# fmazilu/ASR-using-robust-NN

Hardware: AMD Instinct MI355X
Metric: utterances/sec (train, 1 s@16 kHz) (higher is better)
Workload: dtype f32 accumulate, fp16 two-plane split products in the training GEMMs (22-bit operands); 1 GPU; raw 16 kHz waveform -> on-GPU MFCC -> Lipschitz-constrained MLP train step (Adam+NonNeg, simple_norm_constraint rho=0.1), 1xMI355X; global_batch=1024, per_gpu_batch=1024, clip=1 s @ 16 kHz fp32, resident_pool_clips_per_gpu=65536, parallelism=dp1, hip_graph=False

## Files before the change

asr-using-robust-nn_amd/csrc/common.h:

```cpp
#pragma once
#include <hip/hip_runtime.h>
#include <cstdarg>
#include <cstdio>
#include <cstring>
#include <cmath>
#include <algorithm>
#include <vector>
#include "../../include/lipasr.h"

namespace lipasr {

void set_error(const char* fmt, ...);

#define LP_CHECK_ARG(cond, ...)                    \
  do {                                             \
    if (!(cond)) {                                 \
      lipasr::set_error(__VA_ARGS__);              \
      return LIPASR_EINVAL;                        \
    }                                              \
  } while (0)

#define LP_HIP(expr)                                                                   \
  do {                                                                                 \
    hipError_t _e = (expr);                                                            \
    if (_e != hipSuccess) {                                                            \
      lipasr::set_error("%s failed: %s (%s:%d)", #expr, hipGetErrorString(_e), __FILE__, __LINE__); \
      return LIPASR_EHIP;                                                              \
    }                                                                                  \
  } while (0)

#define LP_LAUNCH_CHECK() LP_HIP(hipGetLastError())

bool ensure_dyn_lds(const void* fn, size_t bytes);
int device_cus();
// ... 85 lines not shown
```

asr-using-robust-nn_amd/csrc/core.hip:

```cpp
#include "common.h"
#include <map>
#include <mutex>

namespace lipasr {

static thread_local char g_err[512] = "";

void set_error(const char* fmt, ...) {
  va_list ap;
  va_start(ap, fmt);
  vsnprintf(g_err, sizeof(g_err), fmt, ap);
  va_end(ap);
}

int device_cus() {
  static int cached[16] = {};
  int dev = 0; (void)hipGetDevice(&dev);
  int& c = cached[dev & 15];
  if (!c) { hipDeviceProp_t prop; c = hipGetDeviceProperties(&prop, dev) == hipSuccess ? prop.multiProcessorCount : 256; }
  return c;
}

bool ensure_dyn_lds(const void* fn, size_t bytes) {
  if (bytes <= 48 * 1024) return true;
  struct Limit { size_t granted = 0, refused = SIZE_MAX; };
  static std::mutex mu;
  static std::map<std::pair<const void*, int>, Limit> limits;
  int dev = 0; (void)hipGetDevice(&dev);
  std::lock_guard<std::mutex> lock(mu);
  Limit& l = limits[{fn, dev}];
  if (bytes <= l.granted) return true;
  if (bytes >= l.refused) return false;
  if (hipFuncSetAttribute(fn, hipFuncAttributeMaxDynamicSharedMemorySize, (int)bytes) == hipSuccess) { l.granted = bytes; return true; }
  set_error("hipFuncSetAttribute: %zu bytes of dynamic LDS refused: %s", bytes, hipGetErrorString(hipGetLastError()));
  l.refused = bytes;
  return false;
}

void mfcc_plan_free(MfccPlan* p);
void mlp_plan_free(lipasr_mlp* m);

}

using namespace lipasr;

extern "C" {

int lipasr_version(void) { return 560; }

const char* lipasr_last_error(void) { return g_err; }

int lipasr_create(int device, lipasr_handle_t* out) {
  LP_CHECK_ARG(out != nullptr, "lipasr_create: out is null");
  int n = 0;
  LP_HIP(hipGetDeviceCount(&n));
  LP_CHECK_ARG(device >= 0 && device < n, "lipasr_create: device %d out of range (have %d)", device, n);
  hipDeviceProp_t prop;
  LP_HIP(hipGetDeviceProperties(&prop, device));
  if (strncmp(prop.gcnArchName, "gfx950", 6) != 0) {
    set_error("lipasr_create: device %d is %s; this library is built for gfx950 only", device, prop.gcnArchName);
    return LIPASR_EUNSUPPORTED;
  }
  DeviceGuard g(device);
  if (!g.ok) { set_error("lipasr_create: hipSetDevice(%d) failed", device); return LIPASR_EHIP; }
  lipasr_ctx* c = new lipasr_ctx();
  c->device = device;
  c->scratch_floats = kScratchFloats;
  if (hipMalloc(&c->scratch, c->scratch_floats * sizeof(float)) != hipSuccess) {
    delete c;
    set_error("lipasr_create: scratch allocation failed");
    return LIPASR_ENOMEM;
// ... 55 lines not shown
  LP_HIP(hipEventRecord(h->timers[2 * id], S(stream)));
  return LIPASR_OK;
}

int lipasr_timer_stop(lipasr_handle_t h, int id, lipasr_stream_t stream) {
  LP_CHECK_ARG(h && id >= 0 && (size_t)(2 * id + 1) < h->timers.size(), "lipasr_timer_stop: bad timer id %d", id);
  LP_HIP(hipEventRecord(h->timers[2 * id + 1], S(stream)));
  return LIPASR_OK;
}

int lipasr_timer_elapsed_ms(lipasr_handle_t h, int id, float* ms_host) {
  LP_CHECK_ARG(h && ms_host && id >= 0 && (size_t)(2 * id + 1) < h->timers.size(),
               "lipasr_timer_elapsed_ms: bad argument");
  LP_HIP(hipEventSynchronize(h->timers[2 * id + 1]));
  LP_HIP(hipEventElapsedTime(ms_host, h->timers[2 * id], h->timers[2 * id + 1]));
  return LIPASR_OK;
}

namespace lipasr {
constexpr long long kFlagHardFactor = 4;
__global__ void flag_signal_kernel(int* flag, int value) {
  if (threadIdx.x == 0) __hip_atomic_store(flag, value, __ATOMIC_RELEASE, __HIP_MEMORY_SCOPE_AGENT);
}
__global__ void flag_wait_kernel(const int* flag, int value, int* err, long long soft_ticks) {
  if (threadIdx.x == 0) {
    const long long t0 = wall_clock64();
    bool reported = false;
    while (__hip_atomic_load(flag, __ATOMIC_ACQUIRE, __HIP_MEMORY_SCOPE_AGENT) < value) {
      __builtin_amdgcn_s_sleep(16);
      const long long dt = wall_clock64() - t0;
      if (!reported && dt > soft_ticks) {
        if (__hip_atomic_load(err, __ATOMIC_RELAXED, __HIP_MEMORY_SCOPE_SYSTEM) >= 2) break;
        __hip_atomic_store(err, 1, __ATOMIC_RELAXED, __HIP_MEMORY_SCOPE_SYSTEM);
        reported = true;
      }
      if (dt > kFlagHardFactor * soft_ticks) { __hip_atomic_store(err, 2, __ATOMIC_RELAXED, __HIP_MEMORY_SCOPE_SYSTEM); break; }
    }
  }
}
}

int lipasr_flag_signal(lipasr_handle_t h, int* flag, int value, lipasr_stream_t stream) {
  LP_CHECK_ARG(h && flag, "lipasr_flag_signal: null argument");
  hipLaunchKernelGGL(lipasr::flag_signal_kernel, dim3(1), dim3(64), 0, S(stream), flag, value);
  LP_LAUNCH_CHECK();
  return LIPASR_OK;
}

int lipasr_flag_wait(lipasr_handle_t h, const int* flag, int value, int timeout_ms, int* err, lipasr_stream_t stream) {
  LP_CHECK_ARG(h && flag && err, "lipasr_flag_wait: null argument");
  LP_CHECK_ARG(timeout_ms >= 1 && timeout_ms <= 150000, "lipasr_flag_wait: timeout %d ms outside [1, 150000]", timeout_ms);
  hipLaunchKernelGGL(lipasr::flag_wait_kernel, dim3(1), dim3(64), 0, S(stream), flag, value, err, (long long)timeout_ms * 100000LL);
  LP_LAUNCH_CHECK();
  return LIPASR_OK;
}

int lipasr_graph_begin(lipasr_handle_t h, lipasr_stream_t stream) {
  LP_CHECK_ARG(h != nullptr, "lipasr_graph_begin: null handle");
  LP_HIP(hipStreamBeginCapture(S(stream), hipStreamCaptureModeThreadLocal));
  return LIPASR_OK;
}

int lipasr_graph_end(lipasr_handle_t h, lipasr_stream_t stream, int* graph_id) {
  LP_CHECK_ARG(h && graph_id, "lipasr_graph_end: null argument");
  hipGraph_t graph = nullptr;
  LP_HIP(hipStreamEndCapture(S(stream), &graph));
  hipGraphExec_t exec = nullptr;
  hipError_t e = hipGraphInstantiate(&exec, graph, nullptr, nullptr, 0);
  (void)hipGraphDestroy(graph);
  if (e != hipSuccess) {
    set_error("hipGraphInstantiate failed: %s", hipGetErrorString(e));
// ... 49 lines not shown
```

asr-using-robust-nn_amd/csrc/gemm.hip:

```cpp
#include "gemm.h"
#include <algorithm>
#include <cstdint>

namespace lipasr {

static GemmKnobs g_knobs;
const GemmKnobs& gemm_knobs() { return g_knobs; }
constexpr int kEpiCount = EPI_DH_BNX + 1;
static long g_gemm_launches[GK_KINDS][2][2][2][3][kEpiCount] = {};
static long g_group_launches[3][3] = {};
static long g_group_ring_problems[4] = {};
static long g_group_ring_launches[4] = {};

static int arith_index(int bf16) { return bf16 == 2 ? 2 : bf16 == 1 ? 1 : 0; }
static const GemmTable& gemm_table() { static const GemmTable t; return t; }

static GemmPick gemm_instance(int kind, bool exchange, int amode, int bmode, int ar) {
  const GemmTable& t = gemm_table();
  const GemmShape& s = t.shape[kind];
  return GemmPick{kind, s.tile_m, s.tile_n, s.threads, s.lds_bytes, t.fn[kind][exchange ? 1 : 0][amode][bmode][ar]};
}

static bool aligned16(const void* p) { return (reinterpret_cast<uintptr_t>(p) & 15) == 0; }
static bool ring_legal(int amode, int bmode, const GemmArgs& g) {
// ... 167 lines not shown
using namespace lipasr;

extern "C" {

long lipasr_debug_gemm_launches(int kind, int exchange, int amode, int bmode, int arith, int epi) {
  if (kind < 0 || kind >= GK_KINDS || (exchange | amode | bmode) & ~1 || arith < 0 || arith > 2 || epi < -1 || epi >= kEpiCount) return -1;
  if (!gemm_table().fn[kind][exchange][amode][bmode][arith]) return -1;
  const long* c = g_gemm_launches[kind][exchange][amode][bmode][arith];
  if (epi >= 0) return c[epi];
  long n = 0;
  for (int e = 0; e < kEpiCount; ++e) n += c[e];
  return n;
}

long lipasr_debug_group_launches(int family, int arith, int variant) {
  if (family < 0 || family > 2 || arith < 0 || arith > 2) return -1;
  if (family < 2) return variant == -1 ? g_group_launches[family][arith] : -1;
  if (arith != 2 || variant < -1 || variant > 3) return -1;
  return variant == -1 ? g_group_launches[2][2] : g_group_ring_problems[variant];
}

long lipasr_debug_launch_count(int kind) {
  if (kind == 0) return lipasr_debug_gemm_launches(GK_RING2, 1, 0, 0, 2, -1) + lipasr_debug_gemm_launches(GK_RING2, 1, 0, 1, 2, -1);
  return kind == 1 ? g_group_ring_launches[2] : -1;
}

int lipasr_debug_gemm_mode(int mode) {
  GemmKnobs k;
  k.gemm_mode = mode & 3;
  k.split_dw0 = (mode >> 2) & 1;
  k.group_lds = !((mode >> 3) & 1);
  k.xcd_map = (mode >> 4) & 1;
  k.no_ring = (mode >> 5) & 1;
  k.ring_tile = ((mode >> 6) & 1) ? 1 : ((mode >> 7) & 1) ? 3 : 2;
  k.ring2 = !((mode >> 8) & 1);
  k.ring_x1 = !((mode >> 9) & 1);
  g_knobs = k;
  return LIPASR_OK;
}

static int gemm_entry(const char* fn, lipasr_handle_t h, int arith, int transA, int transB, int M, int N, int K, const float* A, int lda,
                      const float* B, int ldb, float* C, int ldc, float scale_a, float scale_b, lipasr_stream_t stream) {
  LP_CHECK_ARG(h && A && B && C, "%s: null argument", fn);
  LP_CHECK_ARG(arith >= 0 && arith <= 2, "%s: arithmetic mode %d (0 = exact fp32, 1 = bf16 operands, 2 = fp16 two-plane split)", fn, arith);
  LP_CHECK_ARG(M > 0 && N > 0 && K > 0, "%s: empty problem %dx%dx%d", fn, M, N, K);
  LP_CHECK_ARG(lda >= (transA ? M : K) && ldb >= (transB ? K : N) && ldc >= N, "%s: leading dimension too small", fn);
// ... 30 lines not shown
```

asr-using-robust-nn_amd/csrc/stft_bdft.hip:

```cpp
#include "stft.h"

namespace lipasr {

using namespace tables;

typedef _Float16 bd_h8 __attribute__((ext_vector_type(8)));
typedef _Float16 bd_h2 __attribute__((ext_vector_type(2)));
typedef float bd_f2 __attribute__((ext_vector_type(2)));
typedef float bd_f32x16 __attribute__((ext_vector_type(16)));

constexpr int kBdPlane = 1028;
constexpr int kBdSlot = 2 * kBdPlane;
constexpr int kBdSlots = 7;
constexpr int kBdTwF4 = 16 * 64;
constexpr int kBdLdsFloats = kBdSlots * kBdSlot + 4 * kBdTwF4;
constexpr int kBdDummy = 2048;
constexpr double kBdSig = 2048.0, kBdTap = 64.0, kBdMid = 1.0 / 1024.0;
constexpr float kBdOut = 8192.0f;

struct BdftArgs {
  StftArgs st;
  const uint4* cfrag;
  const uint4* efrag;
  const float4* tw;
  const float* wlo;
  const float* whi;
  const unsigned long long* smask;
  const int4* mpos;
  int seg_frames;
  int L;
  const float4* dct_frag;
  const double* aff_mean;
  const double* aff_scale;
  float* out;
};

__device__ __forceinline__ void bd_split8(const float (&x)[8], bd_h8& hi, bd_h8& lo) {
  unsigned h[4], l[4];
#pragma unroll
  for (int i = 0; i < 4; ++i) h[i] = __builtin_bit_cast(unsigned, __builtin_convertvector((bd_f2){x[2 * i], x[2 * i + 1]}, bd_h2));
  asm("v_fma_mixlo_f16 %0, %4, 1.0, -%12 op_sel_hi:[0,0,1]\n\t"
// ... 190 lines not shown
    float pl_, ph_;
    if (j == 0) {
      pl_ = 0.0f; ph_ = 0.0f;
    } else {
      asm("v_cndmask_b32 %0, %1, 0, %2" : "=v"(pl_) : "v"(cl_), "s"(sm[j]));
      asm("v_cndmask_b32 %0, %1, 0, %2" : "=v"(ph_) : "v"(ch_), "s"(sm[j]));
    }
    cl_ = fmaf(wl[j], pw[j], pl_);
    ch_ = fmaf(wh[j], pw[j], ph_);
    sl[j] = cl_; sh[j] = ch_;
  }
}

__device__ __forceinline__ void bd_load_weights(const BdftArgs& a, int lane, float (&wl)[16], float (&wh)[16]) {
#pragma unroll
  for (int q = 0; q < 4; ++q) {
    const float4 l4 = reinterpret_cast<const float4*>(a.wlo)[4 * lane + q], h4 = reinterpret_cast<const float4*>(a.whi)[4 * lane + q];
    wl[4 * q] = l4.x; wl[4 * q + 1] = l4.y; wl[4 * q + 2] = l4.z; wl[4 * q + 3] = l4.w;
    wh[4 * q] = h4.x; wh[4 * q + 1] = h4.y; wh[4 * q + 2] = h4.z; wh[4 * q + 3] = h4.w;
  }
}

__device__ __forceinline__ float bd_frame_finish(const BdftArgs& a, float* __restrict__ stg, const float (&sl)[16], const float (&sh)[16],
                                                 const unsigned (&mp)[6], int lane, int u, int f) {
  const int x = (lane >> 2) & 3;
#pragma unroll
  for (int q = 0; q < 4; ++q) {
    *reinterpret_cast<float4*>(stg + 16 * lane + 4 * (q ^ x)) = make_float4(sl[4 * q], sl[4 * q + 1], sl[4 * q + 2], sl[4 * q + 3]);
    *reinterpret_cast<float4*>(stg + 1024 + 16 * lane + 4 * (q ^ x)) = make_float4(sh[4 * q], sh[4 * q + 1], sh[4 * q + 2], sh[4 * q + 3]);
  }
  if (lane == 0) stg[kBdDummy] = 0.0f;
  const float m0 = ((stg[mp[0] & 0xffff] + stg[mp[0] >> 16]) + stg[mp[1] & 0xffff]) + ((stg[mp[1] >> 16] + stg[mp[2] & 0xffff]) + stg[mp[2] >> 16]);
  const float m1 = ((stg[mp[3] & 0xffff] + stg[mp[3] >> 16]) + stg[mp[4] & 0xffff]) + ((stg[mp[4] >> 16] + stg[mp[5] & 0xffff]) + stg[mp[5] >> 16]);
  const float d0 = 10.0f * log10f(fmaxf(1e-10f, m0)), d1 = 10.0f * log10f(fmaxf(1e-10f, m1));
  float* dbp = a.st.db + ((size_t)u * a.st.n_frames + f) * 128;
  dbp[lane] = d0;
  dbp[lane + 64] = d1;
  const float mx = bd_wave_max(fmaxf(d0, d1));
  if (lane == 0) a.st.fmax[(size_t)u * a.st.n_frames + f] = mx;
  return mx;
}

template <int NT>
__device__ __forceinline__ void bd_dct_epilogue(const BdftArgs& a, float* __restrict__ dbs, float* __restrict__ red, int tid, int u, int nf, float clip_max) {
  const int lane = tid & 63, wave = tid >> 6, li = lane & 31, h = lane >> 5;
  const int L = a.L;
  const int chunk = min(64, (L + 3) & ~3), tp = chunk + 1;
  const int tl = min(chunk, L), tu = max(0, min(nf, tl));
  __builtin_amdgcn_s_waitcnt(0x0f70);
  lds_barrier2();
  if (lane == 0) red[wave] = clip_max;
  __syncthreads();
  float mxall = red[0];
#pragma unroll
  for (int w = 1; w < NT / 64; ++w) mxall = fmaxf(mxall, red[w]);
  const float thr = mxall - 80.0f;
  const float* src = a.st.db + (size_t)u * a.st.n_frames * 128;
  const int n_live = tu * 128;
  constexpr int NJ = 64 * 128 / NT;
  float stage[NJ];
#pragma unroll
  for (int j = 0; j < NJ; ++j) {
    const int i = tid + NT * j;
    stage[j] = (i < n_live) ? __builtin_nontemporal_load(src + i) : 0.0f;
  }
  float4 av4[16];
  const float4* ap = a.dct_frag + (li * 2 + h) * 16;
  if (wave < 2) {
#pragma unroll
    for (int s4 = 0; s4 < 16; ++s4) av4[s4] = ap[s4];
  }
#pragma unroll
  for (int j = 0; j < NJ; ++j) {
    const int i = tid + NT * j, t = i >> 7;
    if (t < chunk) dbs[(i & 127) * tp + t] = (i < n_live) ? fmaxf(stage[j], thr) : 0.0f;
  }
  __syncthreads();
  if (wave < 2) {
    bd_f32x16 acc;
#pragma unroll
    for (int q = 0; q < 16; ++q) acc[q] = 0.0f;
    const float* bp = dbs + h * tp + min(wave * 32 + li, chunk - 1);
#pragma unroll
    for (int s4 = 0; s4 < 16; ++s4) {
      const float a4[4] = {av4[s4].x, av4[s4].y, av4[s4].z, av4[s4].w};
#pragma unroll
      for (int e = 0; e < 4; ++e) acc = __builtin_amdgcn_mfma_f32_32x32x2f32(a4[e], bp[2 * (4 * s4 + e) * tp], acc, 0, 0, 0);
    }
    const int t = wave * 32 + li;
    const int n_out = kNMfcc * L;
    if (t < tl) {
#pragma unroll
      for (int q = 0; q < 16; ++q) {
        const int c = (q & 3) + 8 * (q >> 2) + 4 * h;
        if (c < kNMfcc) {
          float v = (t < tu) ? acc[q] : 0.0f;
          const int oo = c * L + t;
          if (a.aff_mean) v = (float)(((double)v - a.aff_mean[oo]) / a.aff_scale[oo]);
          a.out[(size_t)u * n_out + oo] = v;
        }
      }
    }
  }
}

__device__ __forceinline__ void bd_clip(const BdftArgs& a, int u, int& n_y, int& n_vy, int& n_frames) {
  n_y = a.st.n_y; n_frames = a.st.n_frames; n_vy = a.st.n_y;
  if (a.st.n_valid) {
    clip_lengths(min(max(a.st.n_valid[u], 0), a.st.n_samp_max), a.st.sr_in, &n_vy, &n_y, &n_frames);
    n_frames = min(n_frames, a.st.n_frames);
  }
}

__global__ __launch_bounds__(256) __attribute__((amdgpu_waves_per_eu(2, 2))) void stft_bdft_kernel(BdftArgs a) {
  extern __shared__ __attribute__((aligned(16))) float bd_lds[];
  float* ring = bd_lds;
  float4* twl = reinterpret_cast<float4*>(bd_lds + kBdSlots * kBdSlot);
  const int tid = threadIdx.x, lane = tid & 63;
  const int wave = __builtin_amdgcn_readfirstlane(tid >> 6);
  const int li = lane & 31, h = lane >> 5;
  const int u = blockIdx.y;
  int n_y, n_vy, n_frames;
  bd_clip(a, u, n_y, n_vy, n_frames);
  const int F0 = blockIdx.x * a.seg_frames;
  if (F0 >= n_frames && a.L <= 0) return;
  const int F1 = min(F0 + a.seg_frames, n_frames);
  BdConst K;
  bd_load_const(a, lane, K);
  unsigned long long sm[16];
#pragma unroll
  for (int j = 0; j < 16; ++j) sm[j] = a.smask[j];
#pragma unroll
  for (int i = 0; i < kBdTwF4 / 256; ++i) twl[tid + 256 * i] = a.tw[tid + 256 * i];
  __syncthreads();
  const float* yu = a.st.y + (size_t)u * a.st.n_y;
  const int n_iter = (F0 < n_frames) ? (F1 - F0 + 3) >> 2 : -1;
  unsigned mp[6];
  bd_load_mpos(a, lane, mp);
  float clip_max = -INFINITY;
  float ys[8];
#pragma unroll
  for (int i = 0; i < 8; ++i) ys[i] = 0.0f;
  if (wave >= 1 && n_iter >= 0) bd_fetch(yu, F0 + wave - 1, li, h, n_y, n_vy, ys);
  for (int it = -1; it < n_iter; ++it) {
    const int rel = 4 * it + wave + 3;
    const int jg = F0 + rel;
    const bool do_block = rel >= 0 && jg <= F1 + 2;
    bd_h8 ah, al;
    if (do_block) bd_data_planes(ys, ah, al);
    if (jg + 4 <= F1 + 2) bd_fetch(yu, jg + 4, li, h, n_y, n_vy, ys);
    if (do_block) bd_block(ah, al, K, twl, ring + (rel % kBdSlots) * kBdSlot, lane);
    const int fr = 4 * it + wave, f = F0 + fr;
    const bool do_frame = it >= 0 && f < F1;
    lds_barrier2();
    float sl[16], sh[16];
    if (do_frame) {
      float wl[16], wh[16];
      bd_load_weights(a, lane, wl, wh);
      const float* sb[4];
#pragma unroll
      for (int b = 0; b < 4; ++b) sb[b] = ring + ((fr + b) % kBdSlots) * kBdSlot;
      bd_frame_scan(sb, wl, wh, sm, lane, sl, sh);
    }
    lds_barrier2();
    if (do_frame) {
      const float mx = bd_frame_finish(a, ring + (fr % kBdSlots) * kBdSlot, sl, sh, mp, lane, u, f);
      clip_max = fmaxf(clip_max, mx);
    }
  }
  if (a.L <= 0) return;
  bd_dct_epilogue<256>(a, ring, ring + 128 * 65, tid, u, n_frames, clip_max);
}

static void bd_planes(const double (&v)[8], unsigned int* hi4, unsigned int* lo4) {
  unsigned short hi[8], lw[8];
  for (int j = 0; j < 8; ++j) {
    const _Float16 a = (_Float16)v[j];
    const _Float16 b = (_Float16)(v[j] - (double)a);
    memcpy(&hi[j], &a, 2);
    memcpy(&lw[j], &b, 2);
  }
  for (int w = 0; w < 4; ++w) {
    hi4[w] = (unsigned int)hi[2 * w] | ((unsigned int)hi[2 * w + 1] << 16);
    lo4[w] = (unsigned int)lw[2 * w] | ((unsigned int)lw[2 * w + 1] << 16);
  }
}

template <typename T>
static int bd_upload(T** dptr, const void* src, size_t bytes) {
  LP_HIP(hipMalloc(reinterpret_cast<void**>(dptr), bytes));
  LP_HIP(hipMemcpy(*dptr, src, bytes, hipMemcpyHostToDevice));
  return LIPASR_OK;
}

// ... 71 lines not shown
      if (e0 < s0) continue;
      int n = 0;
      int* dst = &mpos[((size_t)m * 2 + part) * 4];
      dst[n++] = swz(e0) + 1024 * part;
      for (int c = (e0 >> 4) - 1; c >= (s0 >> 4); --c) {
        if (n >= 3) { set_error("lipasr_mfcc_plan: a mel run spans more than three 16-bin groups"); return LIPASR_EUNSUPPORTED; }
        dst[n++] = swz(16 * c + 15) + 1024 * part;
      }
    }
  }
  int rc;
  if ((rc = bd_upload(&t->cfrag, cf.data(), cf.size() * 4)) != LIPASR_OK || (rc = bd_upload(&t->efrag, ef.data(), ef.size() * 4)) != LIPASR_OK ||
      (rc = bd_upload(&t->tw, tw.data(), tw.size() * 4)) != LIPASR_OK || (rc = bd_upload(&t->wlo, wlo.data(), wlo.size() * 4)) != LIPASR_OK ||
      (rc = bd_upload(&t->whi, whi.data(), whi.size() * 4)) != LIPASR_OK || (rc = bd_upload(&t->smask, smask.data(), smask.size() * 8)) != LIPASR_OK ||
      (rc = bd_upload(&t->mpos, mpos.data(), mpos.size() * 4)) != LIPASR_OK) {
    bdft_tables_free(t);
    return rc;
  }
  return LIPASR_OK;
}

bool bdft_can_fuse_dct(int n_frames, int seg_frames, int L) {
  seg_frames = std::max(4, (seg_frames + 3) & ~3);
  return seg_frames >= n_frames && n_frames <= 64 && L >= 1 && L <= 64;
}

int launch_stft_bdft(const StftArgs& st, const BdftTables& t, int batch, int seg_frames, const BdftDct* dct, hipStream_t stream) {
  BdftArgs a;
  a.st = st;
  a.L = 0; a.dct_frag = nullptr; a.aff_mean = nullptr; a.aff_scale = nullptr; a.out = nullptr;
  if (dct && bdft_can_fuse_dct(st.n_frames, seg_frames, dct->L)) {
    a.L = dct->L; a.dct_frag = dct->dct_frag; a.aff_mean = dct->aff_mean; a.aff_scale = dct->aff_scale; a.out = dct->out;
  }
  a.cfrag = t.cfrag; a.efrag = t.efrag; a.tw = t.tw; a.wlo = t.wlo; a.whi = t.whi; a.smask = t.smask; a.mpos = t.mpos;
  seg_frames = std::max(4, (seg_frames + 3) & ~3);
  a.seg_frames = seg_frames;
  const size_t lds = (size_t)kBdLdsFloats * sizeof(float);
  LP_DYN_LDS(stft_bdft_kernel, lds);
  hipLaunchKernelGGL(stft_bdft_kernel, dim3((st.n_frames + seg_frames - 1) / seg_frames, batch), dim3(256), lds, stream, a);
  LP_LAUNCH_CHECK();
  return LIPASR_OK;
}

}
```

asr-using-robust-nn_amd/csrc/stft_mel.hip:

```cpp
#include "mfcc_plan.h"

namespace lipasr {

using namespace tables;


__global__ __launch_bounds__(256) void stft_mel_kernel(StftArgs a) {
  __shared__ __attribute__((aligned(16))) float2 buf[kFftLds];
  __shared__ float wmax[4];
  __shared__ float2 rsum[2][128];
  const int tid = threadIdx.x;
  int u, fp;
  {
    const int npairs = gridDim.x, L = blockIdx.y * gridDim.x + blockIdx.x;
    const int nb = gridDim.y;
    const int full = (nb / 8) * 8 * npairs;
    if (L < full) {
      const int xcd = L & 7, chunk = L >> 3;
      u = (chunk / npairs) * 8 + xcd;
      fp = chunk % npairs;
    } else {
      u = blockIdx.y;
      fp = blockIdx.x;
    }
// ... 506 lines not shown
  if (t < tl) {
#pragma unroll
    for (int q = 0; q < 16; ++q) {
      const int c = (q & 3) + 8 * (q >> 2) + 4 * h;
      if (c < kNMfcc) {
        float v = (t < tu) ? acc[q] : 0.0f;
        const int oo = c * L + t0 + t;
        if (aff_mean) v = (float)(((double)v - aff_mean[oo]) / aff_scale[oo]);
        out[(size_t)u * n_out + oo] = v;
      }
    }
  }
}

std::vector<float> dct_fragments() {
  const std::vector<float> d = tables::dct_matrix();
  std::vector<float> f((size_t)32 * 2 * 64, 0.0f);
  for (int li = 0; li < kNMfcc; ++li)
    for (int h = 0; h < 2; ++h)
      for (int s = 0; s < 64; ++s) f[((size_t)li * 2 + h) * 64 + s] = d[(size_t)li * 128 + 2 * s + h];
  return f;
}

int launch_dct(const MfccPlan* p, int batch, int L, const double* am, const double* as, float* out, const int* n_valid,
                      hipStream_t st) {
  const int chunk = std::min(kDctFrames, (L + 3) & ~3);
  const size_t lds = (size_t)128 * (chunk + 1) * sizeof(float);
  hipLaunchKernelGGL(dct_kernel, dim3(batch, (L + chunk - 1) / chunk), dim3(128), lds, st, p->d_db, p->d_fmax, p->n_frames, L, chunk,
                     reinterpret_cast<const float4*>(p->d_dct), am, as, out, n_valid, p->n_samp, p->sr_in);
  LP_LAUNCH_CHECK();
  return LIPASR_OK;
}

void fill_stft_args(const MfccPlan* p, const float* y, StftArgs* a) {
  a->y = y; a->n_y = p->n_y; a->n_frames = p->n_frames; a->hann = p->d_hann;
  a->tw = reinterpret_cast<const float2*>(p->d_tw);
  a->mel_wlo = p->d_mel_wlo; a->mel_whi = p->d_mel_whi; a->mel_start = p->d_mel_pstart; a->mel_len = p->d_mel_plen;
  a->db = p->d_db; a->fmax = p->d_fmax;
  a->stage_mask = p->stage_mask;
  a->n_valid = nullptr; a->sr_in = p->sr_in; a->n_samp_max = p->n_samp;
}

int launch_from_22k(const MfccPlan* p, MfccPath::Stft kind, const float* y, const int* n_valid, int batch, int L, const double* am,
                    const double* as, float* out, hipStream_t st, hipEvent_t mid, bool stft_only) {
  StftArgs a;
  fill_stft_args(p, y, &a);
  a.n_valid = n_valid;
  switch (kind) {
// ... 39 lines not shown
```

asr-using-robust-nn_amd/lipasr/_native.py:

```python
from __future__ import annotations

import ctypes as C
import os

import torch

_HERE = os.path.dirname(os.path.abspath(__file__))
LIB_PATH = os.environ.get("LIPASR_LIBRARY") or os.path.join(_HERE, "liblipasr.so")

if not os.path.exists(LIB_PATH):
    raise ImportError(
        f"{LIB_PATH} not found: build it with `python asr-using-robust-nn_amd/build.py` "
        "(or __graft_entry__.build()).  lipasr has no CPU fallback."
    )

lib = C.CDLL(LIB_PATH)

OK, EINVAL, ENOMEM, EHIP, EUNSUPPORTED, ESTATE = 0, -1, -2, -3, -4, -5
MAX_LAYERS = 16
SEG_W, SEG_B, SEG_GAMMA, SEG_BETA, SEG_MMEAN, SEG_MVAR = range(6)

c_f = C.c_void_p
c_h = C.c_void_p
c_s = C.c_void_p
# ... 79 lines not shown
    "lipasr_mfcc_plan_dims": (i32, [c_h, PI, PI, PI]),
    "lipasr_mfcc_extract": (i32, [c_h, c_f, i32, c_f, i32, i32, c_f, c_f, c_f, c_s]),
    "lipasr_mfcc_plan_resample": (i32, [c_h, c_f, i32, c_f, c_s]),
    "lipasr_mfcc_plan_from_22k": (i32, [c_h, c_f, i32, i32, i32, c_f, c_f, c_f, c_s]),
    "lipasr_mfcc_plan_vjp": (i32, [c_h, c_f, i32, i32, i32, c_f, c_f, c_f, i32, c_s]),
    "lipasr_mfcc_plan_resample_vjp": (i32, [c_h, c_f, i32, c_f, c_s]),
    "lipasr_mfcc_plan_vjp_short": (i32, [c_h, c_f, i32, i32, i32, c_f, c_f, c_f, i32, c_s]),
    "lipasr_mfcc_plan_vjp_ragged": (i32, [c_h, c_f, i32, c_f, i32, i32, i32, c_f, c_f, c_f, i32, c_s]),
    "lipasr_mfcc_plan_resample_ragged": (i32, [c_h, c_f, i32, c_f, i32, c_f, c_s]),
    "lipasr_mfcc_plan_from_22k_ragged": (i32, [c_h, c_f, c_f, i32, i32, c_f, c_f, c_f, c_s]),
    "lipasr_mfcc_plan_profile_begin": (i32, [c_h, i32]),
    "lipasr_mfcc_plan_profile_end": (i32, [c_h, C.POINTER(f32), PI]),
    "lipasr_mfcc_plan_set": (i32, [c_h, i32, i32]),
    "lipasr_mfcc_profile_begin": (i32, [c_h, i32]),
    "lipasr_mfcc_profile_end": (i32, [c_h, C.POINTER(f32), PI]),
    "lipasr_add_noise_f32": (i32, [c_h, c_f, i32, i32, i32, f32, f32, u64, c_s]),
    "lipasr_debug_set": (i32, [c_h, i32, i32]),
    "lipasr_debug_gemm_mode": (i32, [i32]),
    "lipasr_debug_launch_count": (C.c_long, [i32]),
    "lipasr_debug_gemm_launches": (C.c_long, [i32, i32, i32, i32, i32, i32]),
    "lipasr_debug_group_launches": (C.c_long, [i32, i32, i32]),
    "lipasr_debug_gemm": (i32, [c_h, i32, i32, i32, i32, i32, i32, c_f, i32, c_f, i32, c_f, i32, f32, f32, c_s]),
    "lipasr_flag_signal": (i32, [c_h, C.c_void_p, i32, c_s]),
    "lipasr_flag_wait": (i32, [c_h, C.c_void_p, i32, i32, C.c_void_p, c_s]),
    "lipasr_debug_chain_head": (i32, [i32]),
    "lipasr_debug_table": (i32, [i32, i32, C.POINTER(f32), i32]),
}

SINCE = {"lipasr_mlp_adam_project_product_signal": 560}
lib.lipasr_version.restype = i32
_VERSION = lib.lipasr_version()


def has(name) -> bool:
    return _VERSION >= SINCE.get(name, 0)


for _name, (_res, _args) in PROTOTYPES.items():
    if not has(_name):
        continue
    _fn = getattr(lib, _name)
    _fn.restype = _res
    _fn.argtypes = _args


if os.environ.get("LIPASR_CHAIN_HEAD"):
    lib.lipasr_debug_chain_head(int(os.environ["LIPASR_CHAIN_HEAD"]))
if os.environ.get("LIPASR_GEMM_MODE"):
    lib.lipasr_debug_gemm_mode(int(os.environ["LIPASR_GEMM_MODE"]))


def last_error() -> str:
# ... 156 lines not shown
```

asr-using-robust-nn_amd/lipasr/pipeline.py:

```python
from __future__ import annotations

import ctypes as C

import torch

from . import _native as N
from .extract_features_construct_dataset import MfccExtractor
from .parallel import DataParallel


class TrainPipeline:
    def __init__(self, model, batch, sr_in=16000, n_samp=16000, utterance_length=44, rho=0.1, constraint="product",
                 affine=None, pgd=None, dp=None, use_graph="auto", per_layer_iters=4, extractor=None, mfcc_cus="auto",
                 sync_inputs=True, overlap_buckets=False, sync_bn=False, train_cus="auto"):
        self.sync_inputs = bool(sync_inputs)
        if pgd:
            from .attacks import _norm_value

            self._pgd_norm = _norm_value(pgd.get("norm", float("inf")))
            rinit = int(pgd.get("num_random_init", 0))
            if rinit not in (0, 1):
                raise ValueError(f"pgd num_random_init={rinit}: 0 or 1 (more restarts inside training are not supported)")
            self._pgd_rinit = rinit == 1
            self._pgd_seed = (0xBA11000000000000 + int(model._seed)) & 0xFFFFFFFFFFFFFFFF
# ... 30 lines not shown
        self._gemm_tiles_set = False
        self.stream = torch.cuda.Stream(device=self.dev)
        self.mfcc_stream = self._make_mfcc_stream(mfcc_cus)
        import os as _os

        self._wide_stream = torch.cuda.Stream(device=self.dev) if (self._masked_stream is not None and not self._custom_ex
                                                                  and _os.environ.get("LIPASR_WIDE_WHEN_IDLE", "1") == "1") else None
        self._ev_last_mfcc = None
        self._last_xs = None
        self._last_train_ev = None
        self._n_cu = torch.cuda.get_device_properties(self.dev).multi_processor_count
        self._flags = None
        self._flag_err = None
        want_flags = _os.environ.get("LIPASR_GPU_FLAGS", "auto")
        if want_flags == "auto":
            want_flags = "1" if (self.dp.world == 1 and not self.sync_bn) else "0"
        if want_flags == "1" and self._masked_train_stream is not None:
            self._flags = torch.zeros(2 * self._nbuf, dtype=torch.int32, device=self.dev)
            self._flag_err = torch.zeros(1, dtype=torch.int32).pin_memory()
            self._flag_timeout_ms = int(_os.environ.get("LIPASR_FLAG_TIMEOUT_MS", "30000"))
        self._adam_signal = (self._flags is not None and self.dp.world == 1 and not self.sync_bn and not self.use_graph
                             and self.constraint == "product" and N.has("lipasr_mlp_adam_project_product_signal")
                             and _os.environ.get("LIPASR_ADAM_SIGNAL", "1") == "1")
        self._ev_feat = [torch.cuda.Event() for _ in range(self._nbuf)]
        self._ev_free = [None] * self._nbuf
        self._i = 0
        self._graphs = {}
        self._closed = False
        self._prof = None
        N.register_owner(self)

    def _make_mfcc_stream(self, mfcc_cus):
        import os

        n_cu = torch.cuda.get_device_properties(self.dev).multi_processor_count
        if mfcc_cus == "auto":
            env = os.environ.get("LIPASR_MFCC_CUS")
            if env is not None:
                mfcc_cus = int(env)
            elif self._custom_ex:
                mfcc_cus = (n_cu * 7) // 8
            else:
                rest = self._train_cus == "rest" or (self._train_cus == "auto" and not self.pgd
                                                     and os.environ.get("LIPASR_TRAIN_CUS", "rest") == "rest")
                if rest:
                    mfcc_cus = n_cu // 4 if self.batch <= 768 else ((n_cu * 3) // 8 if self.batch <= 1536 else n_cu // 2)
# ... 214 lines not shown
            self.ex.set(1, self._n_cu)
        if self.sync_inputs:
            xs.wait_stream(caller)
        with torch.cuda.stream(xs):
            if self._flags is not None:
                if self._last_xs is not None and self._last_xs is not xs:
                    xs.wait_stream(self._last_xs)
                self._last_xs = xs
            elif self._ev_last_mfcc is not None and self._wide_stream is not None:
                xs.wait_event(self._ev_last_mfcc)
            if self._flags is not None:
                fl = self._flags
                if self._i > self._nbuf:
                    N.check(N.lib.lipasr_flag_wait(self.h.h, fl[self._nbuf + b:].data_ptr(), self._i - self._nbuf, self._flag_timeout_ms, self._flag_err.data_ptr(), N.stream_ptr()))
            elif self._ev_free[b] is not None:
                xs.wait_event(self._ev_free[b])
            if features is not None:
                self._feats2[b][:bsz].copy_(features)
            else:
                if self._custom_ex:
                    self.ex(waves, self.mean, self.scale, out=self._feats2[b][:bsz])
                else:
                    self.ex(waves, self.L, self.mean, self.scale, out=self._feats2[b][:bsz])
            self._labels2[b][:bsz].copy_(y_onehot)
            if self._flags is not None:
                N.check(N.lib.lipasr_flag_signal(self.h.h, self._flags[b:].data_ptr(), self._i, N.stream_ptr()))
            else:
                self._ev_feat[b].record(xs)
                self._ev_last_mfcc = self._ev_feat[b]
        if wide:
            self.ex.set(1, self.mfcc_cus)
        if self.sync_inputs:
            if self._flags is not None:
                caller.wait_stream(xs)
            else:
                caller.wait_event(self._ev_feat[b])
        with torch.cuda.stream(self.stream):
            self._warm_start()
            if self._flags is not None:
                N.check(N.lib.lipasr_flag_wait(self.h.h, self._flags[b:].data_ptr(), self._i, self._flag_timeout_ms, self._flag_err.data_ptr(), N.stream_ptr()))
            else:
                self.stream.wait_event(self._ev_feat[b])
            prof = None
            if getattr(self, "_prof", None) is not None and self._prof_i < len(self._prof):
                prof = self._prof[self._prof_i]
                self._prof_i += 1
                prof[0].record(self.stream)
            if self.sync_bn:
                self._syncbn_step(bsz, b, gb)
            elif not self.use_graph:
# ... 106 lines not shown
```

include/lipasr.h:

```cpp
#ifndef LIPASR_H
#define LIPASR_H

#include <stddef.h>
#include <stdint.h>

#ifdef __cplusplus
extern "C" {
#endif

#define LIPASR_OK            0
#define LIPASR_EINVAL       -1
#define LIPASR_ENOMEM       -2
#define LIPASR_EHIP         -3
#define LIPASR_EUNSUPPORTED -4
#define LIPASR_ESTATE       -5

#define LIPASR_MAX_LAYERS   16
#define LIPASR_N_MFCC       20
#define LIPASR_N_MELS       128
#define LIPASR_N_FFT        2048
#define LIPASR_HOP          512
#define LIPASR_SR           22050

typedef struct lipasr_ctx* lipasr_handle_t;
typedef struct lipasr_mlp* lipasr_mlp_t;
typedef struct lipasr_mfcc* lipasr_mfcc_t;
typedef void* lipasr_stream_t;

int lipasr_version(void);
const char* lipasr_last_error(void);
int lipasr_create(int device, lipasr_handle_t* out);
int lipasr_destroy(lipasr_handle_t h);

int lipasr_timer_create(lipasr_handle_t h, int* timer_id);
int lipasr_timer_start(lipasr_handle_t h, int timer_id, lipasr_stream_t stream);
int lipasr_timer_stop(lipasr_handle_t h, int timer_id, lipasr_stream_t stream);
int lipasr_timer_elapsed_ms(lipasr_handle_t h, int timer_id, float* ms_host);

int lipasr_flag_signal(lipasr_handle_t h, int* flag, int value, lipasr_stream_t stream);
int lipasr_flag_wait(lipasr_handle_t h, const int* flag, int value, int timeout_ms, int* err, lipasr_stream_t stream);

int lipasr_graph_begin(lipasr_handle_t h, lipasr_stream_t stream);
int lipasr_graph_end(lipasr_handle_t h, lipasr_stream_t stream, int* graph_id);
int lipasr_graph_launch(lipasr_handle_t h, int graph_id, lipasr_stream_t stream);
int lipasr_graph_destroy(lipasr_handle_t h, int graph_id);

int lipasr_stream_create_masked(lipasr_handle_t h, const uint32_t* cu_mask, int n_words, lipasr_stream_t* out);
int lipasr_stream_destroy(lipasr_handle_t h, lipasr_stream_t stream);


int lipasr_sigma_max(lipasr_handle_t h, const float* W, int rows, int cols, float* v_state, int warm,
                     int iters, int clamp_nonneg, float* sigma_out, lipasr_stream_t stream);

int lipasr_project_per_layer(lipasr_handle_t h, float* const* Ws, const int* rows, const int* cols,
                             int n_layers, float rho, float* v_state, int warm, int iters,
                             float* sigmas_out, lipasr_stream_t stream);

int lipasr_project_product(lipasr_handle_t h, float* const* Ws, const int* rows, const int* cols,
                           int n_layers, float rho, const int* order, int n_order,
                           float* norms_out, lipasr_stream_t stream);

int lipasr_product_norm(lipasr_handle_t h, const float* const* Ws, const int* rows, const int* cols,
// ... 192 lines not shown
```

Before: 3.196 million utterances/sec.

## Keep dB frames in registers for fused DCT and add fused label-copy signal

The fused STFT+DCT kernel now keeps each block's log-mel dB values in registers (up to 11 iterations, templated KEEP). The DCT epilogue builds its LDS tile from those registers instead of re-reading dB rows from global memory, and the max reduction uses a reserved LDS slot. The fuse condition is narrowed to n_frames <= 44. Separately, a new opt-in kernel copies the one-hot labels and sets the ready flag in one launch, saving a launch per batch, though it is off by default. A DCT launch counter is also added for debugging; the register arrays raise register pressure.

```diff
diff --git a/asr-using-robust-nn_amd/csrc/common.h b/asr-using-robust-nn_amd/csrc/common.h
--- a/asr-using-robust-nn_amd/csrc/common.h
+++ b/asr-using-robust-nn_amd/csrc/common.h
@@ -10,6 +10,7 @@
 
 namespace lipasr {
 
+extern long g_dct_launches;
 void set_error(const char* fmt, ...);
 
 #define LP_CHECK_ARG(cond, ...)                    \
diff --git a/asr-using-robust-nn_amd/csrc/core.hip b/asr-using-robust-nn_amd/csrc/core.hip
--- a/asr-using-robust-nn_amd/csrc/core.hip
+++ b/asr-using-robust-nn_amd/csrc/core.hip
@@ -46,7 +46,7 @@
 
 extern "C" {
 
-int lipasr_version(void) { return 560; }
+int lipasr_version(void) { return 570; }
 
 const char* lipasr_last_error(void) { return g_err; }
 
@@ -148,6 +148,28 @@
 __global__ void flag_signal_kernel(int* flag, int value) {
   if (threadIdx.x == 0) __hip_atomic_store(flag, value, __ATOMIC_RELEASE, __HIP_MEMORY_SCOPE_AGENT);
 }
+constexpr int kFlagCopyThreads = 256;
+__global__ __launch_bounds__(kFlagCopyThreads) void flag_signal_copy_kernel(int* flag, int value, unsigned char* __restrict__ dst,
+                                                                             const unsigned char* __restrict__ src, size_t n) {
+  const size_t t = threadIdx.x;
+  const uintptr_t both = reinterpret_cast<uintptr_t>(dst) | reinterpret_cast<uintptr_t>(src);
+  size_t done = 0;
+  if ((both & 15) == 0) {
+    const size_t n16 = n / 16;
+#pragma unroll 4
+    for (size_t i = t; i < n16; i += kFlagCopyThreads) reinterpret_cast<uint4*>(dst)[i] = reinterpret_cast<const uint4*>(src)[i];
+    done = n16 * 16;
+  } else if ((both & 3) == 0) {
+    const size_t n4 = n / 4;
+#pragma unroll 4
+    for (size_t i = t; i < n4; i += kFlagCopyThreads) reinterpret_cast<unsigned*>(dst)[i] = reinterpret_cast<const unsigned*>(src)[i];
+    done = n4 * 4;
+  }
+  for (size_t i = done + t; i < n; i += kFlagCopyThreads) dst[i] = src[i];
+  __threadfence();
+  __syncthreads();
+  if (t == 0) __hip_atomic_store(flag, value, __ATOMIC_RELEASE, __HIP_MEMORY_SCOPE_AGENT);
+}
 __global__ void flag_wait_kernel(const int* flag, int value, int* err, long long soft_ticks) {
   if (threadIdx.x == 0) {
     const long long t0 = wall_clock64();
@@ -173,6 +195,16 @@
   return LIPASR_OK;
 }
 
+int lipasr_flag_signal_copy(lipasr_handle_t h, int* flag, int value, void* dst, const void* src, size_t n_bytes, lipasr_stream_t stream) {
+  LP_CHECK_ARG(h && flag, "lipasr_flag_signal_copy: null argument");
+  LP_CHECK_ARG(n_bytes == 0 || (dst && src), "lipasr_flag_signal_copy: null buffer with %zu bytes to copy", n_bytes);
+  LP_CHECK_ARG(n_bytes <= ((size_t)1 << 24), "lipasr_flag_signal_copy: %zu bytes is a copy of its own, not a payload (limit 16 MiB)", n_bytes);
+  hipLaunchKernelGGL(lipasr::flag_signal_copy_kernel, dim3(1), dim3(lipasr::kFlagCopyThreads), 0, S(stream), flag, value,
+                     static_cast<unsigned char*>(dst), static_cast<const unsigned char*>(src), n_bytes);
+  LP_LAUNCH_CHECK();
+  return LIPASR_OK;
+}
+
 int lipasr_flag_wait(lipasr_handle_t h, const int* flag, int value, int timeout_ms, int* err, lipasr_stream_t stream) {
   LP_CHECK_ARG(h && flag && err, "lipasr_flag_wait: null argument");
   LP_CHECK_ARG(timeout_ms >= 1 && timeout_ms <= 150000, "lipasr_flag_wait: timeout %d ms outside [1, 150000]", timeout_ms);
diff --git a/asr-using-robust-nn_amd/csrc/gemm.hip b/asr-using-robust-nn_amd/csrc/gemm.hip
--- a/asr-using-robust-nn_amd/csrc/gemm.hip
+++ b/asr-using-robust-nn_amd/csrc/gemm.hip
@@ -213,6 +213,7 @@
 
 long lipasr_debug_launch_count(int kind) {
   if (kind == 0) return lipasr_debug_gemm_launches(GK_RING2, 1, 0, 0, 2, -1) + lipasr_debug_gemm_launches(GK_RING2, 1, 0, 1, 2, -1);
+  if (kind == 2) return lipasr::g_dct_launches;
   return kind == 1 ? g_group_ring_launches[2] : -1;
 }
 
diff --git a/asr-using-robust-nn_amd/csrc/stft_bdft.hip b/asr-using-robust-nn_amd/csrc/stft_bdft.hip
--- a/asr-using-robust-nn_amd/csrc/stft_bdft.hip
+++ b/asr-using-robust-nn_amd/csrc/stft_bdft.hip
@@ -13,10 +13,11 @@
 constexpr int kBdSlot = 2 * kBdPlane;
 constexpr int kBdSlots = 7;
 constexpr int kBdTwF4 = 16 * 64;
-constexpr int kBdLdsFloats = kBdSlots * kBdSlot + 4 * kBdTwF4;
+constexpr int kBdLdsFloats = kBdSlots * kBdSlot + 4 * kBdTwF4 + 4;
 constexpr int kBdDummy = 2048;
 constexpr double kBdSig = 2048.0, kBdTap = 64.0, kBdMid = 1.0 / 1024.0;
 constexpr float kBdOut = 8192.0f;
+constexpr int kBdKeep = 11;
 
 struct BdftArgs {
   StftArgs st;
@@ -253,7 +254,7 @@
 }
 
 __device__ __forceinline__ float bd_frame_finish(const BdftArgs& a, float* __restrict__ stg, const float (&sl)[16], const float (&sh)[16],
-                                                 const unsigned (&mp)[6], int lane, int u, int f) {
+                                                 const unsigned (&mp)[6], int lane, int u, int f, float& d0, float& d1) {
   const int x = (lane >> 2) & 3;
 #pragma unroll
   for (int q = 0; q < 4; ++q) {
@@ -263,7 +264,8 @@
   if (lane == 0) stg[kBdDummy] = 0.0f;
   const float m0 = ((stg[mp[0] & 0xffff] + stg[mp[0] >> 16]) + stg[mp[1] & 0xffff]) + ((stg[mp[1] >> 16] + stg[mp[2] & 0xffff]) + stg[mp[2] >> 16]);
   const float m1 = ((stg[mp[3] & 0xffff] + stg[mp[3] >> 16]) + stg[mp[4] & 0xffff]) + ((stg[mp[4] >> 16] + stg[mp[5] & 0xffff]) + stg[mp[5] >> 16]);
-  const float d0 = 10.0f * log10f(fmaxf(1e-10f, m0)), d1 = 10.0f * log10f(fmaxf(1e-10f, m1));
+  d0 = 10.0f * log10f(fmaxf(1e-10f, m0));
+  d1 = 10.0f * log10f(fmaxf(1e-10f, m1));
   float* dbp = a.st.db + ((size_t)u * a.st.n_frames + f) * 128;
   dbp[lane] = d0;
   dbp[lane + 64] = d1;
@@ -272,41 +274,39 @@
   return mx;
 }
 
-template <int NT>
-__device__ __forceinline__ void bd_dct_epilogue(const BdftArgs& a, float* __restrict__ dbs, float* __restrict__ red, int tid, int u, int nf, float clip_max) {
+template <int NT, int KEEP>
+__device__ __forceinline__ void bd_dct_epilogue(const BdftArgs& a, float* __restrict__ dbs, float* __restrict__ red, int tid, int u, int nf, float clip_max,
+                                                const float (&k0)[KEEP], const float (&k1)[KEEP]) {
   const int lane = tid & 63, wave = tid >> 6, li = lane & 31, h = lane >> 5;
   const int L = a.L;
   const int chunk = min(64, (L + 3) & ~3), tp = chunk + 1;
   const int tl = min(chunk, L), tu = max(0, min(nf, tl));
-  __builtin_amdgcn_s_waitcnt(0x0f70);
-  lds_barrier2();
-  if (lane == 0) red[wave] = clip_max;
-  __syncthreads();
-  float mxall = red[0];
-#pragma unroll
-  for (int w = 1; w < NT / 64; ++w) mxall = fmaxf(mxall, red[w]);
-  const float thr = mxall - 80.0f;
-  const float* src = a.st.db + (size_t)u * a.st.n_frames * 128;
-  const int n_live = tu * 128;
-  constexpr int NJ = 64 * 128 / NT;
-  float stage[NJ];
-#pragma unroll
-  for (int j = 0; j < NJ; ++j) {
-    const int i = tid + NT * j;
-    stage[j] = (i < n_live) ? __builtin_nontemporal_load(src + i) : 0.0f;
-  }
   float4 av4[16];
   const float4* ap = a.dct_frag + (li * 2 + h) * 16;
   if (wave < 2) {
 #pragma unroll
     for (int s4 = 0; s4 < 16; ++s4) av4[s4] = ap[s4];
   }
-#pragma unroll
-  for (int j = 0; j < NJ; ++j) {
-    const int i = tid + NT * j, t = i >> 7;
-    if (t < chunk) dbs[(i & 127) * tp + t] = (i < n_live) ? fmaxf(stage[j], thr) : 0.0f;
-  }
-  __syncthreads();
+  if (lane == 0) red[wave] = clip_max;
+  lds_barrier2();
+  float mxall = red[0];
+#pragma unroll
+  for (int w = 1; w < NT / 64; ++w) mxall = fmaxf(mxall, red[w]);
+  const float thr = mxall - 80.0f;
+  float* c0 = dbs + lane * tp;
+  float* c1 = dbs + (lane + 64) * tp;
+#pragma unroll
+  for (int k = 0; k < 64 / (NT / 64); ++k) {
+    const int t = (NT / 64) * k + wave;
+    if (k < KEEP && t < tu) {
+      c0[t] = fmaxf(k0[k < KEEP ? k : 0], thr);
+      c1[t] = fmaxf(k1[k < KEEP ? k : 0], thr);
+    } else if (t < chunk) {
+      c0[t] = 0.0f;
+      c1[t] = 0.0f;
+    }
+  }
+  lds_barrier2();
   if (wave < 2) {
     bd_f32x16 acc;
 #pragma unroll
@@ -343,6 +343,7 @@
   }
 }
 
+template <int KEEP>
 __global__ __launch_bounds__(256) __attribute__((amdgpu_waves_per_eu(2, 2))) void stft_bdft_kernel(BdftArgs a) {
   extern __shared__ __attribute__((aligned(16))) float bd_lds[];
   float* ring = bd_lds;
@@ -354,7 +355,7 @@
   int n_y, n_vy, n_frames;
   bd_clip(a, u, n_y, n_vy, n_frames);
   const int F0 = blockIdx.x * a.seg_frames;
-  if (F0 >= n_frames && a.L <= 0) return;
+  if (F0 >= n_frames && KEEP == 0) return;
   const int F1 = min(F0 + a.seg_frames, n_frames);
   BdConst K;
   bd_load_const(a, lane, K);
@@ -369,6 +370,9 @@
   unsigned mp[6];
   bd_load_mpos(a, lane, mp);
   float clip_max = -INFINITY;
+  float k0[KEEP ? KEEP : 1], k1[KEEP ? KEEP : 1];
+#pragma unroll
+  for (int e = 0; e < KEEP; ++e) { k0[e] = 0.0f; k1[e] = 0.0f; }
   float ys[8];
 #pragma unroll
   for (int i = 0; i < 8; ++i) ys[i] = 0.0f;
@@ -395,12 +399,14 @@
     }
     lds_barrier2();
     if (do_frame) {
-      const float mx = bd_frame_finish(a, ring + (fr % kBdSlots) * kBdSlot, sl, sh, mp, lane, u, f);
+      float d0, d1;
+      const float mx = bd_frame_finish(a, ring + (fr % kBdSlots) * kBdSlot, sl, sh, mp, lane, u, f, d0, d1);
       clip_max = fmaxf(clip_max, mx);
-    }
-  }
-  if (a.L <= 0) return;
-  bd_dct_epilogue<256>(a, ring, ring + 128 * 65, tid, u, n_frames, clip_max);
+#pragma unroll
+      for (int e = 0; e < KEEP; ++e) { k0[e] = (it == e) ? d0 : k0[e]; k1[e] = (it == e) ? d1 : k1[e]; }
+    }
+  }
+  if constexpr (KEEP > 0) bd_dct_epilogue<256, KEEP>(a, ring, bd_lds + kBdLdsFloats - 4, tid, u, n_frames, clip_max, k0, k1);
 }
 
 static void bd_planes(const double (&v)[8], unsigned int* hi4, unsigned int* lo4) {
@@ -518,7 +524,7 @@
 
 bool bdft_can_fuse_dct(int n_frames, int seg_frames, int L) {
   seg_frames = std::max(4, (seg_frames + 3) & ~3);
-  return seg_frames >= n_frames && n_frames <= 64 && L >= 1 && L <= 64;
+  return seg_frames >= n_frames && n_frames <= 4 * kBdKeep && L >= 1 && L <= 64;
 }
 
 int launch_stft_bdft(const StftArgs& st, const BdftTables& t, int batch, int seg_frames, const BdftDct* dct, hipStream_t stream) {
@@ -532,8 +538,14 @@
   seg_frames = std::max(4, (seg_frames + 3) & ~3);
   a.seg_frames = seg_frames;
   const size_t lds = (size_t)kBdLdsFloats * sizeof(float);
-  LP_DYN_LDS(stft_bdft_kernel, lds);
-  hipLaunchKernelGGL(stft_bdft_kernel, dim3((st.n_frames + seg_frames - 1) / seg_frames, batch), dim3(256), lds, stream, a);
+  const dim3 grid((st.n_frames + seg_frames - 1) / seg_frames, batch);
+  if (a.L > 0) {
+    LP_DYN_LDS(stft_bdft_kernel<kBdKeep>, lds);
+    hipLaunchKernelGGL(stft_bdft_kernel<kBdKeep>, grid, dim3(256), lds, stream, a);
+  } else {
+    LP_DYN_LDS(stft_bdft_kernel<0>, lds);
+    hipLaunchKernelGGL(stft_bdft_kernel<0>, grid, dim3(256), lds, stream, a);
+  }
   LP_LAUNCH_CHECK();
   return LIPASR_OK;
 }
diff --git a/asr-using-robust-nn_amd/csrc/stft_mel.hip b/asr-using-robust-nn_amd/csrc/stft_mel.hip
--- a/asr-using-robust-nn_amd/csrc/stft_mel.hip
+++ b/asr-using-robust-nn_amd/csrc/stft_mel.hip
@@ -552,8 +552,11 @@
   return f;
 }
 
+long g_dct_launches = 0;
+
 int launch_dct(const MfccPlan* p, int batch, int L, const double* am, const double* as, float* out, const int* n_valid,
                       hipStream_t st) {
+  ++g_dct_launches;
   const int chunk = std::min(kDctFrames, (L + 3) & ~3);
   const size_t lds = (size_t)128 * (chunk + 1) * sizeof(float);
   hipLaunchKernelGGL(dct_kernel, dim3(batch, (L + chunk - 1) / chunk), dim3(128), lds, st, p->d_db, p->d_fmax, p->n_frames, L, chunk,
diff --git a/asr-using-robust-nn_amd/lipasr/_native.py b/asr-using-robust-nn_amd/lipasr/_native.py
--- a/asr-using-robust-nn_amd/lipasr/_native.py
+++ b/asr-using-robust-nn_amd/lipasr/_native.py
@@ -125,12 +125,13 @@
     "lipasr_debug_group_launches": (C.c_long, [i32, i32, i32]),
     "lipasr_debug_gemm": (i32, [c_h, i32, i32, i32, i32, i32, i32, c_f, i32, c_f, i32, c_f, i32, f32, f32, c_s]),
     "lipasr_flag_signal": (i32, [c_h, C.c_void_p, i32, c_s]),
+    "lipasr_flag_signal_copy": (i32, [c_h, C.c_void_p, i32, C.c_void_p, C.c_void_p, C.c_size_t, c_s]),
     "lipasr_flag_wait": (i32, [c_h, C.c_void_p, i32, i32, C.c_void_p, c_s]),
     "lipasr_debug_chain_head": (i32, [i32]),
     "lipasr_debug_table": (i32, [i32, i32, C.POINTER(f32), i32]),
 }
 
-SINCE = {"lipasr_mlp_adam_project_product_signal": 560}
+SINCE = {"lipasr_mlp_adam_project_product_signal": 560, "lipasr_flag_signal_copy": 570}
 lib.lipasr_version.restype = i32
 _VERSION = lib.lipasr_version()
 
diff --git a/asr-using-robust-nn_amd/lipasr/pipeline.py b/asr-using-robust-nn_amd/lipasr/pipeline.py
--- a/asr-using-robust-nn_amd/lipasr/pipeline.py
+++ b/asr-using-robust-nn_amd/lipasr/pipeline.py
@@ -76,6 +76,8 @@
         self._adam_signal = (self._flags is not None and self.dp.world == 1 and not self.sync_bn and not self.use_graph
                              and self.constraint == "product" and N.has("lipasr_mlp_adam_project_product_signal")
                              and _os.environ.get("LIPASR_ADAM_SIGNAL", "1") == "1")
+        self._signal_copy = (self._flags is not None and N.has("lipasr_flag_signal_copy")
+                             and _os.environ.get("LIPASR_SIGNAL_COPY", "0") == "1")
         self._ev_feat = [torch.cuda.Event() for _ in range(self._nbuf)]
         self._ev_free = [None] * self._nbuf
         self._i = 0
@@ -336,10 +338,16 @@
                     self.ex(waves, self.mean, self.scale, out=self._feats2[b][:bsz])
                 else:
                     self.ex(waves, self.L, self.mean, self.scale, out=self._feats2[b][:bsz])
-            self._labels2[b][:bsz].copy_(y_onehot)
-            if self._flags is not None:
+            lab = self._labels2[b][:bsz]
+            if self._flags is not None and self._signal_copy and y_onehot.dtype == lab.dtype and y_onehot.shape == lab.shape \
+                    and y_onehot.device == lab.device and y_onehot.is_contiguous():
+                N.check(N.lib.lipasr_flag_signal_copy(self.h.h, self._flags[b:].data_ptr(), self._i, lab.data_ptr(), y_onehot.data_ptr(),
+                                                      lab.numel() * lab.element_size(), N.stream_ptr()))
+            elif self._flags is not None:
+                lab.copy_(y_onehot)
                 N.check(N.lib.lipasr_flag_signal(self.h.h, self._flags[b:].data_ptr(), self._i, N.stream_ptr()))
             else:
+                lab.copy_(y_onehot)
                 self._ev_feat[b].record(xs)
                 self._ev_last_mfcc = self._ev_feat[b]
         if wide:
diff --git a/include/lipasr.h b/include/lipasr.h
--- a/include/lipasr.h
+++ b/include/lipasr.h
@@ -38,6 +38,8 @@
 int lipasr_timer_elapsed_ms(lipasr_handle_t h, int timer_id, float* ms_host);
 
 int lipasr_flag_signal(lipasr_handle_t h, int* flag, int value, lipasr_stream_t stream);
+int lipasr_flag_signal_copy(lipasr_handle_t h, int* flag, int value, void* dst, const void* src, size_t n_bytes,
+                            lipasr_stream_t stream);
 int lipasr_flag_wait(lipasr_handle_t h, const int* flag, int value, int timeout_ms, int* err, lipasr_stream_t stream);
 
 int lipasr_graph_begin(lipasr_handle_t h, lipasr_stream_t stream);
```

New measurement: 3.207 million utterances/sec (median of 3 runs). No clear change (+0.3%).
